# alphacep/vosk-tts

Measured on AMD Instinct MI355X. Metric: audio_samples_per_sec, higher is better.
Workload: dtype f32

## Files before the change

### vosk_tts_amd/csrc/conv_mfma.hip.h

```cpp
#pragma once
#include <type_traits>
#include <hip/hip_runtime.h>
#include <stdint.h>

typedef float f32x16 __attribute__((ext_vector_type(16)));
typedef float f32x4 __attribute__((ext_vector_type(4)));

#define CONV_CI_T 16
#define CONV_MAX_HALO 64
#define CONV_MAX_GROUPS 3

enum ConvEpilogue {
  EPI_STORE = 0,
  EPI_GATE = 1,
  EPI_RESSKIP = 2,
  EPI_COUPLE = 3,
};

struct ConvGroup {
  const float* x;
  const float* x2;
  const float* x3;
  const float* w;
  const float* w16;
  const void* wb;
  const float* bias;
  float* y;
  float* y2;
  const float* res;
  int K;
  int dil;
  int pad_l;
  int n_sg;
};

struct ConvParams {
  ConvGroup g[CONV_MAX_GROUPS];
  int n_groups;
  int B;
  int Cin;
  int x_ch_off;
  int x_ch_sign;
  long long x_bstride;
  int Tin;
  int Tin_stride;
  int M;
  int Cout;
  int Tout;
  int Tout_stride;
  long long y_bstride;
  float in_slope;
  float in_scale;
  int x_split;
  int in_mask;
  int reflect;
  const int* len;
  int relu;
  const float* scale_b;
  int scale_b_stride;
  int scale_b_off;
  int out_mask;
  const float* bias_b;
  int bias_b_stride;
  int bias_b_off;
  int ups_u;
  int ups_cout;
  int ups_shift[8];
  float* io;
  const float* u;
  float* skip;
  int H;
  int first;
  int last;
  int ntiles_m, ntiles_n;
  int xcd_mode;
  const float* dds_y2; const float* dds_g2; const float* dds_b2;
  const float* dds_sw; const float* dds_sb; const float* dds_g1; const float* dds_b1;
  float* dds_xout;
  int dds_dil;
  const float* dds_z; const float* dds_pw; const float* dds_pb;
  long long dds_z_bstride;
  const float* ln_g; const float* ln_b; const float* ln_base; const float* ln_vec;
  int ln_vec_stride, ln_vec_off;
  float* ln_out;
  const float* ln_stat_in; float* ln_stat_out; int ln_nmb;
  int row_len;
  long long* dbg;
  const int* rag;
  int rag_in_mul, rag_in_add, rag_out_mul, rag_out_add;
  int rag_tab_add;
  int rag_out_cap_add;
  int skip_len;
  const int* tile_start;
};

__device__ __forceinline__ int conv_rag_limit(int rl, int rcap, int mul, int add, int cap_add = 0) {
  const int v = rl * mul + add, c = rcap * mul + cap_add;
  return v < c ? v : c;
}

template <int BYTES>
__device__ __forceinline__ void kernarg_warm() {
  static_assert(BYTES <= 1024, "extend kernarg_warm");
  constexpr int LAST = (BYTES - 1) / 64 * 64;
#define KW_OFF(i) ((i) * 64 < LAST ? (i) * 64 : LAST)
  const unsigned long long kp = (unsigned long long)__builtin_amdgcn_kernarg_segment_ptr();
  int d;
  asm volatile(
      "s_load_dword %0, %1, %2\n s_load_dword %0, %1, %3\n s_load_dword %0, %1, %4\n s_load_dword %0, %1, %5\n"
      "s_load_dword %0, %1, %6\n s_load_dword %0, %1, %7\n s_load_dword %0, %1, %8\n s_load_dword %0, %1, %9\n"
      "s_load_dword %0, %1, %10\n s_load_dword %0, %1, %11\n s_load_dword %0, %1, %12\n s_load_dword %0, %1, %13\n"
      "s_load_dword %0, %1, %14\n s_load_dword %0, %1, %15\n s_load_dword %0, %1, %16\n s_load_dword %0, %1, %17\n"
      "s_waitcnt lgkmcnt(0)"
      : "=&s"(d)
      : "s"(kp), "n"(KW_OFF(0)), "n"(KW_OFF(1)), "n"(KW_OFF(2)), "n"(KW_OFF(3)), "n"(KW_OFF(4)), "n"(KW_OFF(5)), "n"(KW_OFF(6)),
        "n"(KW_OFF(7)), "n"(KW_OFF(8)), "n"(KW_OFF(9)), "n"(KW_OFF(10)), "n"(KW_OFF(11)), "n"(KW_OFF(12)), "n"(KW_OFF(13)),
        "n"(KW_OFF(14)), "n"(KW_OFF(15))
      : "memory");
#undef KW_OFF
}

__device__ __forceinline__ int conv_pair_mtiles(int ntiles_m, int L = blockIdx.x, int nblk = gridDim.x) {
  const int run = 8 * ntiles_m;
  if (ntiles_m < 2 || L >= (nblk / run) * run) return L;
  const int base = L / run * run, r = L - base, x = r & 7, w = r >> 3;
  return base + x * ntiles_m + w;
}
__device__ __forceinline__ bool conv_decode_block(const ConvParams& P, int& mt, int& grp, int& nt, int& b) {
  const int Lb = blockIdx.x;
  if (P.tile_start) {
    int id = conv_pair_mtiles(P.ntiles_m);
    mt = id % P.ntiles_m; id /= P.ntiles_m;
    const int total = P.tile_start[P.B];
    int q;
    if (P.n_groups > 1) { q = id % (P.ntiles_n * P.B); grp = id / (P.ntiles_n * P.B); }
    else { q = id; grp = 0; }
    if (q >= total) return false;
    int lo = 0, hi = P.B - 1;
    while (lo < hi) { const int mid = (lo + hi + 1) >> 1; if (P.tile_start[mid] <= q) lo = mid; else hi = mid - 1; }
    b = lo;
    nt = q - P.tile_start[b];
    return true;
  }
  if (P.xcd_mode == 11) {
    const int x = Lb & 7, w = Lb >> 3;
    const int per = P.ntiles_m * P.ntiles_n, n = (per - x + 7) >> 3;
    const int a = n < 32 ? n : 32;
    const int b7 = 32 - a < n ? 32 - a : n;
    int idx;
    if (w < a) { grp = 0; idx = w; }
    else if (w < a + b7) { grp = 1; idx = w - a; }
    else if (w < a + b7 + n) { grp = 2; idx = w - a - b7; }
    else if (w < a + 2 * n) { grp = 1; idx = w - a - n; }
    else { grp = 0; idx = w - 2 * n; }
    if (idx >= n) return false;
    const int t = idx * 8 + x;
    mt = t % P.ntiles_m; nt = t / P.ntiles_m;
    b = 0;
    return true;
  }
  int id;
  {
    const int nblk = gridDim.x, L = Lb;
    const int q = nblk >> 3, r = nblk & 7, xcd = L & 7, within = L >> 3;
    id = (xcd < r ? xcd * (q + 1) : r * (q + 1) + (xcd - r) * q) + within;
  }
  if (P.n_groups > 1) {
    id = P.B > 1 ? conv_pair_mtiles(P.ntiles_m) : Lb;
    mt = id % P.ntiles_m; id /= P.ntiles_m;
    nt = id % P.ntiles_n; id /= P.ntiles_n;
    b = id % P.B;
    grp = id / P.B;
  } else {
    mt = id % P.ntiles_m; id /= P.ntiles_m;
    nt = id % P.ntiles_n;
// ... 406 lines not shown
#pragma unroll
        for (int ni = 0; ni < NI; ++ni)
          acc[mi][ni] = __builtin_amdgcn_mfma_f32_32x32x2f32(a[cur][mi][p >> 2][p & 3], bv[p][ni], acc[mi][ni], 0, 0, 0);
    __builtin_amdgcn_sched_barrier(0);
  };
  using slot0 = std::integral_constant<int, 0>;
  using slot1 = std::integral_constant<int, 1>;

  for (int c = 0; c < nchunks; ++c) {
    CONV_DBG_DO(if (P.dbg) dbg_x = __builtin_readcyclecounter();)
    const float* lb = lds + (c & 1) * (CONV_CI_T * ROW) + h * ROW + wn * (NI * 32) + l31 + tap_base;
    tap(slot0{}, lb, 0);
    if (c + 1 < nchunks) load_chunk(c + 1);
    __builtin_amdgcn_sched_barrier(0);
    int kk = 1;
#pragma unroll 1
    for (; kk + 1 < K; kk += 2) {
      tap(slot1{}, lb, kk);
      tap(slot0{}, lb, kk + 1);
    }
    if (kk < K) {
      tap(slot1{}, lb, kk);
    } else {
#pragma unroll
      for (int mi = 0; mi < MI; ++mi) {
        a[0][mi][0] = a[1][mi][0];
        a[0][mi][1] = a[1][mi][1];
      }
    }
    CONV_DBG_DO(if (P.dbg) { const long long t_ = __builtin_readcyclecounter(); dbg_tap += t_ - dbg_x; dbg_x = t_; })
    if (c + 1 < nchunks) store_chunk((c + 1) & 1);
    __syncthreads();
    CONV_DBG_DO(if (P.dbg) dbg_sync += __builtin_readcyclecounter() - dbg_x;)
  }
  CONV_DBG_DO(if (P.dbg && blockIdx.x == 0 && lane == 0) {
    P.dbg[wave * 8 + 1] = dbg_tap;
    P.dbg[wave * 8 + 2] = dbg_sync;
    P.dbg[wave * 8 + 3] = __builtin_readcyclecounter() - dbg_t0;
  })

  const int lenb = (P.out_mask || EPI == EPI_RESSKIP || EPI == EPI_COUPLE) ? P.len[b] : 0x7fffffff;
  if (EPI == EPI_GATE) {
    const int j = (m0 >> 6) + wm;
#pragma unroll
    for (int ni = 0; ni < NI; ++ni)
#pragma unroll
      for (int e0 = 0; e0 < 16; e0 += 4) {
        float at[4], as[4];
#pragma unroll
        for (int i = 0; i < 4; ++i) { at[i] = acc[0][ni][e0 + i]; as[i] = acc[MI - 1][ni][e0 + i]; }
        conv_epilogue_gate<4>(P, G, b, j * 32 + 4 * h, e0, n0 + wn * (NI * 32) + ni * 32 + l31, at, as);
      }
    BT_BLOCK_END();
    return;
  }
  if (EPI == EPI_STORE && conv_epilogue_store_fast_ok(P, G)) {
    conv_epilogue_store_fragments<MI, NI>(P, G, b, lenb, m0 + wm * MI * 32, n0 + wn * (NI * 32), h, l31, acc);
    CONV_DBG_DO(if (P.dbg && blockIdx.x == 0 && lane == 0) P.dbg[wave * 8 + 4] = __builtin_readcyclecounter() - dbg_t0;)
    BT_BLOCK_END();
    return;
  }
#pragma unroll
  for (int mi = 0; mi < MI; ++mi) {
#pragma unroll
    for (int ni = 0; ni < NI; ++ni) {
#pragma unroll
      for (int e0 = 0; e0 < 16; e0 += 4) {
        float v[4];
#pragma unroll
        for (int i = 0; i < 4; ++i) v[i] = acc[mi][ni][e0 + i];
        conv_epilogue_frag<EPI, 4>(P, G, b, lenb, m0 + (wm * MI + mi) * 32 + 4 * h, e0, n0 + wn * (NI * 32) + ni * 32 + l31, v);
      }
    }
  }
  CONV_DBG_DO(if (P.dbg && blockIdx.x == 0 && lane == 0) P.dbg[wave * 8 + 4] = __builtin_readcyclecounter() - dbg_t0;)
  BT_BLOCK_END();
}

__device__ __forceinline__ float ks_ld(const float* base, unsigned byte_off) {
  return *reinterpret_cast<const float*>(reinterpret_cast<const char*>(base) + byte_off);
}
struct ks_true { static constexpr bool value = true; };
struct ks_false { static constexpr bool value = false; };
template <int MI, int NI, int EPI, int NIN, int NW>
__global__ void __launch_bounds__(NW * 64) conv_mfma_ks_kernel(const ConvParams P) {
  constexpr int M_T = MI * 32;
  constexpr int N_T = NI * 32;
  constexpr int NE = 16 / NW;
  extern __shared__ float lds[];
  kernarg_warm<sizeof(ConvParams)>();

  const int tid = threadIdx.x, lane = tid & 63;
  const int wave = __builtin_amdgcn_readfirstlane(tid >> 6);
  const int h = lane >> 5, l31 = lane & 31;
  CONV_DBG(0);
  int mt, grp, nt, b;
  if (!conv_decode_block(P, mt, grp, nt, b)) return;
  const ConvGroup& G = P.g[grp];

  const int n0 = nt * N_T, m0 = mt * M_T;
  const int K = G.K, dil = G.dil;
  int tap_base = 0;
  if (P.ups_u) tap_base = P.ups_shift[m0 / P.ups_cout];
  const int nchunks = P.Cin / CONV_CI_T;
  int t_lim = P.Tin;
  if (P.in_mask) { int lb = P.len[b]; t_lim = lb < t_lim ? lb : t_lim; }
  if (P.rag) {
    const int rl = P.rag[b], rc = P.rag[P.B];
    if (n0 >= conv_rag_limit(rl, rc, P.rag_out_mul, P.rag_out_add, P.rag_out_cap_add)) return;
    const int il = conv_rag_limit(rl, rc, P.rag_in_mul, P.rag_in_add);
    t_lim = il < t_lim ? il : t_lim;
  }
  if (P.skip_len && n0 >= P.len[b]) return;
  const float in_scale = P.in_scale, in_slope = P.in_slope;

  int tcol[NI];
#pragma unroll
  for (int ni = 0; ni < NI; ++ni) tcol[ni] = n0 + ni * 32 + l31 - G.pad_l + tap_base;
  const long long rs = (long long)P.x_ch_sign * P.Tin_stride;
  const long long ubase = (long long)b * P.x_bstride + (long long)P.x_ch_off * P.Tin_stride + (rs < 0 ? rs : 0);
  const unsigned hoff = (unsigned)(h ? (rs < 0 ? 0 : rs) : (rs < 0 ? -rs : 0));
  const float* xu = G.x + ubase;
  const float* xu2 = G.x2 ? G.x2 + ubase : nullptr;
  const float* xu3 = G.x3 ? G.x3 + ubase : nullptr;

  f32x16 acc[MI][NI];
#pragma unroll
  for (int mi = 0; mi < MI; ++mi)
#pragma unroll
    for (int ni = 0; ni < NI; ++ni)
#pragma unroll
      for (int e = 0; e < 16; ++e) acc[mi][ni][e] = 0.f;

  const int n_mblocks = P.M >> 5;
  const f32x4* wp[MI];
#pragma unroll
  for (int mi = 0; mi < MI; ++mi) {
    int mb = (m0 >> 5) + mi;
    if (mb >= n_mblocks) mb = 0;
    wp[mi] = reinterpret_cast<const f32x4*>(G.w) + (size_t)mb * G.n_sg * 64;
  }
  const int total_taps = nchunks * K;
  const int my_taps = wave < total_taps ? (total_taps - wave + NW - 1) / NW : 0;
  const int q_last = wave + NW * (my_taps > 0 ? my_taps - 1 : 0);
  const int c_last = q_last / K, k_last = q_last - c_last * K;

  constexpr int KS_U = NW >= 16 ? 1 : (NW == 8 ? (MI * NI > 1 ? 2 : 4) : 4);
  struct TapBuf {
    f32x4 a[KS_U][MI][2];
    float bq[KS_U][8][NI];
    unsigned ok[KS_U];
  };
  int lc = wave / K, lk = wave - (wave / K) * K;
  int lq = wave;
  const int step_c = NW / K, step_k = NW - step_c * K;
  const unsigned lane16 = (unsigned)lane * 16u;
  const float* xq2 = NIN > 2 ? xu2 : xu;
  const float* xq3 = NIN > 2 ? (xu3 ? xu3 : xu2) : xu;
  const float s3 = (NIN > 2 && xu3) ? 1.f : 0.f;
  const int split_chunk = NIN == 2 ? P.x_split / CONV_CI_T : 0x7fffffff;
  const int refl_t = P.reflect ? ((P.Tin > 1) ? 1 : 0) : -1;

  auto pipe_step = [&](auto has_cur, auto act, const TapBuf& cur, TapBuf& nxt) {
#pragma unroll
    for (int u = 0; u < KS_U; ++u) {
      const bool live = lq <= q_last;
      const int cc = live ? lc : c_last;
      const int kc = live ? lk : k_last;
      const int sg = 2 * (cc * K + kc);
      const bool second = NIN == 2 && cc >= split_chunk;
      const float* xsrc = second ? xu2 : xu;
      const long long coff = (long long)(second ? cc - split_chunk : cc) * CONV_CI_T * rs;
      unsigned lo[NI];
      unsigned okb = 0;
#pragma unroll
      for (int ni = 0; ni < NI; ++ni) {
        int t = tcol[ni] + kc * dil;
        t = (t == -1 && refl_t >= 0) ? refl_t : t;
        okb |= ((t >= 0) & (t < t_lim) & live) ? (1u << ni) : 0u;
        lo[ni] = (hoff + (unsigned)(t < 0 ? 0 : (t >= P.Tin ? P.Tin - 1 : t))) * 4u;
      }
      nxt.ok[u] = okb;
#pragma unroll
      for (int mi = 0; mi < MI; ++mi) {
        nxt.a[u][mi][0] = *reinterpret_cast<const f32x4*>(reinterpret_cast<const char*>(wp[mi] + (size_t)sg * 64) + lane16);
        nxt.a[u][mi][1] = *reinterpret_cast<const f32x4*>(reinterpret_cast<const char*>(wp[mi] + (size_t)(sg + 1) * 64) + lane16);
      }
#pragma unroll
      for (int p = 0; p < 8; ++p) {
        const long long ro = coff + 2 * p * rs;
#pragma unroll
        for (int ni = 0; ni < NI; ++ni) {
          float v = ks_ld(xsrc + ro, lo[ni]);
          if (NIN > 2) v = (v + ks_ld(xq2 + ro, lo[ni]) + s3 * ks_ld(xq3 + ro, lo[ni])) * in_scale;
          nxt.bq[u][p][ni] = v;
        }
        if (decltype(has_cur)::value) {
          bool okb_[NI];
#pragma unroll
          for (int ni = 0; ni < NI; ++ni) okb_[ni] = (cur.ok[u] >> ni) & 1u;
#pragma unroll
          for (int ni = 0; ni < NI; ++ni) {
            const float x_ = cur.bq[u][p][ni];
            const float bv = okb_[ni] ? (decltype(act)::value ? fmaxf(x_, x_ * in_slope) : x_) : 0.f;
#pragma unroll
            for (int mi = 0; mi < MI; ++mi)
              acc[mi][ni] = __builtin_amdgcn_mfma_f32_32x32x2f32(cur.a[u][mi][p >> 2][p & 3], bv, acc[mi][ni], 0, 0, 0);
          }
        }
        __builtin_amdgcn_sched_barrier(0);
      }
      lq += NW;
      lk += step_k;
      lc += step_c + (lk >= K ? 1 : 0);
      lk -= lk >= K ? K : 0;
    }
  };

  CONV_DBG(1);
  auto run_pipe = [&](auto act) {
    TapBuf t0, t1;
    pipe_step(ks_false{}, act, t1, t0);
#pragma unroll 1
    for (int tp = 0; tp < my_taps; tp += 2 * KS_U) {
      pipe_step(ks_true{}, act, t0, t1);
      if (tp + KS_U < my_taps) pipe_step(ks_true{}, act, t1, t0);
    }
  };
  if (my_taps > 0) {
    if (in_slope == 1.f) run_pipe(ks_false{});
    else run_pipe(ks_true{});
  }
  CONV_DBG(2);

  float* red = lds;
#pragma unroll
  for (int mi = 0; mi < MI; ++mi)
#pragma unroll
    for (int ni = 0; ni < NI; ++ni)
#pragma unroll
      for (int e = 0; e < 16; ++e) red[(((wave * MI + mi) * NI + ni) * 16 + e) * 64 + lane] = acc[mi][ni][e];
  __syncthreads();
  CONV_DBG(3);
  const int lenb = (P.out_mask || EPI == EPI_RESSKIP || EPI == EPI_COUPLE) ? P.len[b] : 0x7fffffff;
  float sum[MI][NI][NE];
#pragma unroll
  for (int mi = 0; mi < MI; ++mi)
#pragma unroll
    for (int ni = 0; ni < NI; ++ni)
#pragma unroll
      for (int ee = 0; ee < NE; ++ee) {
        const int e = NE * wave + ee;
        float a = 0.f;
#pragma unroll
        for (int w = 0; w < NW; ++w) a += red[(((w * MI + mi) * NI + ni) * 16 + e) * 64 + lane];
        sum[mi][ni][ee] = a;
      }
  CONV_DBG(4);
#pragma unroll
  for (int ni = 0; ni < NI; ++ni) {
    const int col = n0 + ni * 32 + l31;
    if (EPI == EPI_GATE) {
      conv_epilogue_gate<NE>(P, G, b, (m0 >> 6) * 32 + 4 * h, NE * wave, col, sum[0][ni], sum[MI - 1][ni]);
    } else {
#pragma unroll
      for (int mi = 0; mi < MI; ++mi) conv_epilogue_frag<EPI, NE>(P, G, b, lenb, m0 + mi * 32 + 4 * h, NE * wave, col, sum[mi][ni]);
    }
  }
  CONV_DBG(5);
}

template <typename F>
static void pack_conv_weights(float* dst, int Mpad, int Cin, int K, F src ) {
  const int n_sg = Cin / CONV_CI_T * 2 * K;
  for (int mb = 0; mb < Mpad / 32; ++mb)
    for (int sg = 0; sg < n_sg; ++sg)
      for (int lane = 0; lane < 64; ++lane)
        for (int s4 = 0; s4 < 4; ++s4) {
          const int S = sg * 4 + s4;
          const int chunk = S / (8 * K), within = S % (8 * K);
          const int kk = within / 8, p = within % 8;
          const int ci = chunk * CONV_CI_T + 2 * p + (lane >> 5);
          const int row = mb * 32 + (lane & 31);
          dst[(((size_t)mb * n_sg + sg) * 64 + lane) * 4 + s4] = src(row, ci, kk);
        }
}
```

### vosk_tts_amd/csrc/conv_small.hip.h

```cpp
#pragma once
#include "conv_mfma.hip.h"

#define C16_MAXU 20

template <typename F>
static void pack_conv_weights16(float* dst, int Mpad16, int Cin, int K, F src) {
  const int n_u = Cin / CONV_CI_T * K;
  for (int mb = 0; mb < Mpad16 / 16; ++mb)
    for (int u = 0; u < n_u; ++u)
      for (int lane = 0; lane < 64; ++lane)
        for (int q = 0; q < 4; ++q) {
          const int chunk = u / K, kk = u % K;
          const int ci = chunk * CONV_CI_T + 4 * q + (lane >> 4);
          const int row = mb * 16 + (lane & 15);
          dst[(((size_t)mb * n_u + u) * 64 + lane) * 4 + q] = src(row, ci, kk);
        }
}

static inline int c16_row_pitch(int row) { return row <= 16 ? 16 : (row <= 48 ? 48 : 80); }

#define DDS_MAXI 16
#define DDS_XP 36
__device__ __forceinline__ float c16_gelu(float v) { return 0.5f * v * (1.0f + erff(v * 0.70710678118654752440f)); }
template <int NG, int NC>
// ... 410 lines not shown
#pragma unroll
  for (int r = 0; r < 4; ++r) red[(wave * 4 + r) * 64 + lane] = acc0[r] + acc1[r];
  __syncthreads();
  if (EPI == EPI_GATE) {
    if (tid >= 128) return;
    const int ch = tid >> 4, col = n0 + (tid & 15);
    float at = 0.f, as = 0.f;
#pragma unroll
    for (int w = 0; w < NW; ++w) {
      at += red[(w * 4 + (ch & 3)) * 64 + (ch >> 2) * 16 + (tid & 15)];
      as += red[(w * 4 + (ch & 3)) * 64 + ((ch >> 2) + 2) * 16 + (tid & 15)];
    }
    const int c = mt * 8 + ch;
    const float tv = tanhf(at + ep0 + ep2);
    const float sv = 1.0f / (1.0f + __expf(-(as + ep1 + ep3)));
    if (col < P.Tout && c < P.H) G.y[(long long)b * P.y_bstride + (long long)c * P.Tout_stride + col] = tv * sv;
    return;
  }
  const bool want_stat = EPI == EPI_STORE && P.ln_stat_out != nullptr;
  if (tid >= 256 && !want_stat) return;
  const bool act = tid < 256;
  const int row = (tid >> 4) & 15, col = n0 + (tid & 15);
  float v = 0.f;
#pragma unroll
  for (int w = 0; w < NW; ++w) v += red[(w * 4 + (row & 3)) * 64 + (row >> 2) * 16 + (tid & 15)];
  const int r = m0 + row;
  const bool ok = act && col < P.Tout && r < P.Cout;
  if (!ok && !want_stat) return;
  if (EPI == EPI_STORE) {
    v += ep0;
    v += ep1;
    if (P.relu == 1) v = v > 0.f ? v : 0.f;
    else if (P.relu == 2) v = v / (1.0f + __expf(-v));
    else if (P.relu == 3) v = 0.5f * v * (1.0f + erff(v * 0.70710678118654752440f));
    if (P.out_mask && col >= lenb) v = 0.f;
    v *= ep2;
    v += ep3;
    const long long o = (long long)b * P.y_bstride + (long long)r * P.Tout_stride + col;
    if (ok) {
      G.y[o] = v;
      if (G.y2) G.y2[o] = v;
    }
    CONV_DBG(5);
    if (want_stat) {
      float* st = lds + NW * 4 * 64;
      const int nrow = P.Cout - m0 < 16 ? P.Cout - m0 : 16;
      float sv = ok ? v : 0.f;
      sv += __shfl_xor(sv, 16, 64);
      sv += __shfl_xor(sv, 32, 64);
      if (act && lane < 16) st[wave * 16 + lane] = sv;
      __syncthreads();
      const int c15 = tid & 15;
      const float mean = (st[c15] + st[16 + c15] + st[32 + c15] + st[48 + c15]) / (float)nrow;
      const float d = ok ? v - mean : 0.f;
      float q = d * d;
      q += __shfl_xor(q, 16, 64);
      q += __shfl_xor(q, 32, 64);
      __syncthreads();
      if (act && lane < 16) st[wave * 16 + lane] = q;
      __syncthreads();
      if (tid < 16 && col < P.Tout) {
        float* dst = P.ln_stat_out + (((long long)b * P.ln_nmb + mt) * P.Tout + col) * 2;
        dst[0] = mean;
        dst[1] = st[c15] + st[16 + c15] + st[32 + c15] + st[48 + c15];
      }
    }
  } else if (EPI == EPI_RESSKIP) {
    const bool to_skip = P.last || r >= P.H;
    const int sr = (P.last || r < P.H) ? r : r - P.H;
    const bool valid = col < lenb;
    float o = ep1 + v + ep0;
    if (to_skip) { if (P.last && !valid) o = 0.f; }
    else if (!valid) o = 0.f;
    float* dst = to_skip ? P.skip : P.io;
    dst[(long long)b * P.y_bstride + (long long)sr * P.Tout_stride + col] = o;
  } else {
    const long long bo = (long long)b * P.y_bstride + col;
    P.io[bo + (long long)(P.H + r) * P.Tout_stride] = col < lenb ? (ep1 - (v + ep0)) : 0.f;
    P.io[bo + (long long)r * P.Tout_stride] = ep2;
  }
}

#define WP_PITCH 96
typedef float f32x4u __attribute__((ext_vector_type(4), aligned(4)));
template <int V> struct wp_int { static constexpr int value = V; };
template <int NW, int KT>
__device__ __forceinline__ void conv_wp_body(const ConvParams& P, const ConvGroup& G, float* lds, int mt, int nt, int b, int wave, int lane) {
  constexpr int NE = 16 / NW;
  const int h = lane >> 5, l31 = lane & 31;
  const int n0 = nt * 32, m0 = mt * 32;
  const int K = KT ? KT : G.K, dil = G.dil;
  const int nchunks = P.Cin / CONV_CI_T;
  const int my_chunks = wave < nchunks ? (nchunks - wave + NW - 1) / NW : 0;
  const int last_c = wave + NW * (my_chunks > 0 ? my_chunks - 1 : 0);
  int mb = m0 >> 5;
  if (mb >= (P.M >> 5)) mb = 0;
  const f32x4* wp = reinterpret_cast<const f32x4*>(G.w) + (size_t)mb * G.n_sg * 64 + lane;
  f32x4 a[2][2];
  int lci = 0, lk = 0;
  auto load_a_half = [&](f32x4 (&d)[2], int half) {
    const int c = wave + NW * lci;
    const bool live = c <= last_c && my_chunks > 0;
    const size_t sg = 2 * ((size_t)(live ? c : last_c) * K + (live ? lk : K - 1));
    d[half] = wp[(sg + half) * 64];
    if (half) {
      ++lk;
      if (lk == K) { lk = 0; ++lci; }
    }
  };
  auto load_a = [&](f32x4 (&d)[2]) { load_a_half(d, 0); load_a_half(d, 1); };
  load_a(a[0]);
  load_a(a[1]);
  int bi = b;
  asm volatile("" : "+v"(bi));
  int len_raw = 0x7fffffff, rag_raw = 0x7fffffff;
  if (P.in_mask || P.out_mask || P.skip_len) len_raw = P.len[bi];
  int rag_cap = 0x7fffffff;
  if (P.rag) { rag_raw = P.rag[bi]; rag_cap = P.rag[P.B]; }

  const int row_len = 32 + (K - 1) * dil;
  const int nvec = (row_len + 3) >> 2;
  const bool two = nvec > 16;
  const int t_base = n0 - G.pad_l;
  const int r4 = lane >> 4, v16 = lane & 15;
  int tvp[2], tcp[2];
#pragma unroll
  for (int ps = 0; ps < 2; ++ps) {
    tvp[ps] = t_base + 4 * (v16 + 16 * ps);
    const int tc = tvp[ps] < 0 ? 0 : tvp[ps];
    tcp[ps] = tc > P.Tin - 4 ? P.Tin - 4 : tc;
  }
  const unsigned lrow = (unsigned)(r4 * P.Tin_stride);
  float* sl = lds + wave * (CONV_CI_T * WP_PITCH);
  float* sw = sl + r4 * WP_PITCH + 4 * v16;
  const float* xb = G.x + (long long)b * P.x_bstride;
  const float slope = P.in_slope;
  f32x4 v0[4], v1[4];
  const float* xb2 = G.x2 ? G.x2 + (long long)b * P.x_bstride : xb;
  const int split_chunk = P.x_split ? P.x_split / CONV_CI_T : 0x7fffffff;
  auto load_slab = [&](int ci) {
    const int c = wave + NW * ci;
    const float* xc = c >= split_chunk ? xb2 + (long long)(c - split_chunk) * CONV_CI_T * P.Tin_stride : xb + (long long)c * CONV_CI_T * P.Tin_stride;
#pragma unroll
    for (int j = 0; j < 4; ++j)
      v0[j] = *reinterpret_cast<const f32x4u*>(reinterpret_cast<const char*>(xc + 4 * j * P.Tin_stride) + (lrow + (unsigned)tcp[0]) * 4u);
    if (two) {
#pragma unroll
      for (int j = 0; j < 4; ++j)
        v1[j] = *reinterpret_cast<const f32x4u*>(reinterpret_cast<const char*>(xc + 4 * j * P.Tin_stride) + (lrow + (unsigned)tcp[1]) * 4u);
    }
  };
  if (my_chunks > 0) load_slab(0);
  const int ecol = n0 + l31;
  const int ecolc = ecol < P.Tout ? ecol : P.Tout - 1;
  long long eoff[NE];
  bool eok[NE];
  float ebias[NE], eres[NE];
#pragma unroll
  for (int i = 0; i < NE; ++i) {
    const int e = NE * wave + i;
    const int r = m0 + 4 * h + (e & 3) + 8 * (e >> 2);
    const int rc = r < P.Cout ? r : P.Cout - 1;
    eok[i] = ecol < P.Tout && r < P.Cout;
    eoff[i] = (long long)b * P.y_bstride + (long long)rc * P.Tout_stride + ecolc;
    const float bv = (G.bias ? G.bias : G.w)[rc];
    const float rv = (G.res ? G.res : G.y)[eoff[i]];
    ebias[i] = G.bias ? bv : 0.f;
// ... 168 lines not shown
```

### vosk_tts_amd/csrc/engine_convplan.hip.h

```cpp
#pragma once
struct ConvSelect {
  int force_tile = 0;
  int ks_waves = 0;
  int wp_mode = 0;
  int sp_mode = -1;
  int no_bf3 = 0;
  long env_ks_threshold = 512;
  int env_ks_shape = 0;
  long env_big_blocks = 512;
  int env_ks_waves = 0;
  int env_wp_mode = 0;
  int ks_force() const { return ks_waves ? ks_waves : env_ks_waves; }
  int wp() const { return wp_mode ? wp_mode : env_wp_mode; }
  int sp() const { return sp_mode >= 0 ? sp_mode : 1; }
};
static ConvSelect conv_select_env() {
  ConvSelect e;
  if (const char* v = getenv("VITS_KS_THRESHOLD")) e.env_ks_threshold = atol(v);
  if (const char* v = getenv("VITS_KS_SHAPE")) e.env_ks_shape = atoi(v);
  if (const char* v = getenv("VITS_BIG_BLOCKS")) e.env_big_blocks = atol(v);
  if (const char* v = getenv("VITS_KS_WAVES")) e.env_ks_waves = atoi(v);
  if (const char* v = getenv("VITS_CONV_WP")) e.env_wp_mode = atoi(v);
  return e;
}
static ConvSelect& conv_select() {
  static const ConvSelect env = conv_select_env();
  static thread_local ConvSelect sel = env;
  return sel;
}

enum ConvFamily { CONV_BIG, CONV_KS, CONV_C16, CONV_WP, CONV_SP, CONV_BF3 };
struct ConvPlan {
  ConvFamily family;
  int epi;
  int WM, WN, MI, NI;
  int NW;
  int NIN;
  int MAXU, PRO;
  int JT;
  int M_T, N_T;
};
static ConvPlan plan_big(int WM, int WN, int MI, int NI, int epi) { return {CONV_BIG, epi, WM, WN, MI, NI, WM * WN, 1, 0, 0, 0, WM * MI * 32, WN * NI * 32}; }
static ConvPlan plan_bf3(int MI, int epi) { return {CONV_BF3, epi, 2, 2, MI, 2, 4, 1, 0, 0, 0, 64 * MI, 128}; }
static ConvPlan plan_sp(int epi, int halo) { return {CONV_SP, epi, 2, 2, 1, 1, 4, 1, 0, 0, halo ? 2 : 1, 64, 64}; }
static ConvPlan plan_wp() { return {CONV_WP, EPI_STORE, 1, 1, 1, 1, 8, 1, 0, 0, 0, 32, 32}; }
static ConvPlan plan_c16_dds() { return {CONV_C16, EPI_STORE, 1, 1, 1, 1, 8, 1, 8, 1, 0, 16, 16}; }

static std::string conv_plan_name(const ConvPlan& p) {
  static const char* const epi[4] = {"STORE", "GATE", "RESSKIP", "COUPLE"};
  char b[64];
  switch (p.family) {
    case CONV_BIG: snprintf(b, sizeof b, "conv_mfma_kernel<%d,%d,%d,%d,%s>", p.WM, p.WN, p.MI, p.NI, epi[p.epi]); break;
    case CONV_KS: snprintf(b, sizeof b, "conv_mfma_ks_kernel<%d,%d,%s,%d,%d>", p.MI, p.NI, epi[p.epi], p.NIN, p.NW); break;
    case CONV_C16:
      if (p.PRO == 1) snprintf(b, sizeof b, "conv16_kernel<STORE,dds>");
      else if (p.PRO) snprintf(b, sizeof b, "conv16_kernel<STORE,ln,%d>", p.NW);
      else snprintf(b, sizeof b, "conv16_kernel<%s,%d>", epi[p.epi], p.NW);
      break;
    case CONV_WP: snprintf(b, sizeof b, "conv_wp_kernel<%d>", p.NW); break;
    case CONV_SP: snprintf(b, sizeof b, "conv_sp_kernel<%s>", epi[p.epi]); break;
    case CONV_BF3: snprintf(b, sizeof b, p.epi == EPI_GATE ? "conv_bf3_kernel<%d,GATE>" : "conv_bf3_kernel<%d>", p.MI); break;
  }
  return b;
}

static int ks_pick_waves(const ConvParams& P, long nblk, const ConvSelect& sel) {
  const int force = sel.ks_force();
  if (force == 4 || force == 8 || force == 16) return force;
  int taps = 0;
  for (int g = 0; g < P.n_groups; ++g) { const int t = P.Cin / CONV_CI_T * P.g[g].K; if (t > taps) taps = t; }
  if (nblk <= 1024 && taps >= 32) return 16;
  if (nblk <= 2048 && taps >= 16) return 8;
  return 4;
}
static int c16_waves(const ConvParams& P, int epi) {
  const ConvGroup& G = P.g[0];
  if (P.n_groups != 1 || !G.w16 || P.ups_u || G.x3 || (G.x2 && !P.x_split) || P.reflect || P.rag || P.Cin % CONV_CI_T) return 0;
  if (epi == EPI_GATE && (P.H % 8)) return 0;
  const int halo = (G.K - 1) * G.dil;
  if (halo > 48) return 0;
  if (P.ln_g && P.Cin > 8 * C16_LN_MAXC) return 0;
  if (P.ln_g && (halo > 16 || P.in_slope != 1.f || P.in_scale != 1.f || P.x_split || P.x_ch_sign != 1 || P.x_ch_off || epi != EPI_STORE)) return 0;
  const size_t lds = ((size_t)P.Cin * c16_row_pitch(16 + halo) + 16 * 32) * sizeof(float);
  if (lds > 150 * 1024) return 0;
  const int units = P.Cin / CONV_CI_T * G.K;
  if (units <= 4 * C16_MAXU) return 4;
  if (units <= 8 * C16_MAXU) return 8;
  return 0;
}
static constexpr long C16_COLS_DDS = 800;
static bool c16_dds_ok(const ConvParams& P, int dds_K, const ConvSelect& sel) {
  return (sel.force_tile == 0 || sel.force_tile == 3) && (long)P.B * P.Tout <= C16_COLS_DDS && P.g[0].w16 && P.g[0].K == 1 && P.Cin % 32 == 0 &&
         P.Cin <= 16 * DDS_MAXI && dds_K == 3 && P.Cin / CONV_CI_T <= 8 * 8 && P.len && (!P.dds_sw || P.dds_dil <= 9);
}
static bool conv_wp_ok(const ConvParams& P, int epi, int halo, bool small, const ConvSelect& sel) {
  const int mode = sel.wp();
  if (mode == 1 || epi != EPI_STORE) return false;
  if (P.x_ch_sign != 1 || P.x_ch_off || P.tile_start || P.ups_u || P.reflect || P.in_scale != 1.f || P.ln_g || P.dds_y2 || P.ln_stat_out) return false;
  if (P.Cin % CONV_CI_T || P.Tin < 4 || 32 + halo > WP_PITCH || P.in_slope < 0.f || P.in_slope > 1.f) return false;
  if (P.x_split && (P.n_groups != 1 || P.x_split % CONV_CI_T || !P.g[0].x2)) return false;
  for (int g = 0; g < P.n_groups; ++g)
    if (P.g[g].x3 || (P.g[g].x2 && !P.x_split)) return false;
  if (mode == 2) return true;
  return small && P.Cin >= 8 * CONV_CI_T && (long)P.B * P.Tout >= 256;
}
// ... 85 lines not shown
```

### vosk_tts_amd/csrc/engine_launch.hip.h

```cpp
#pragma once
static std::atomic<int> g_launch_log{0};
static std::mutex g_launch_log_mu;
static std::map<std::string, int> g_launch_counts;
struct ProfScope {
  vits_session* s; bool on; bool log; const char* op; std::string lk;
  ProfScope(vits_session* s_, const char* name, double flops, const char* kernel = "-")
      : s(s_), on(s_->profile), log(g_launch_log.load(std::memory_order_relaxed) != 0), op(name) {
    if (log) lk = kernel;
    if (!on) return;
    ProfRec r; r.name = name; r.kernel = kernel; r.flops = flops;
    hipEventCreate(&r.e0); hipEventCreate(&r.e1);
    hipEventRecord(r.e0, s->stream);
    s->prof.push_back(r);
  }
  void set_kernel(const char* k) { if (on) s->prof.back().kernel = k; if (log) lk = k; }
  ~ProfScope() {
    if (on) hipEventRecord(s->prof.back().e1, s->stream);
    if (log) { std::lock_guard<std::mutex> g(g_launch_log_mu); ++g_launch_counts[std::string(op) + "|" + lk]; }
  }
};


static bool big_lds_needed(std::atomic<unsigned long long>& done);
static void persist_launch(vits_session* s, vits_session::PersistProg& pp, const char* name, const float* d_noise = nullptr, float nsw = 0.f,
                           uint64_t seed = 0, const int64_t* d_ids = nullptr, const int* d_forced = nullptr, float length_scale = 1.f,
                           float noise_scale = 0.f) {
  vits_model* m = s->m;
  ProfScope ps(s, name, pp.flops, "persist_kernel");
  PCall c;
  c.ctl = s->ps_ctl; c.ids = reinterpret_cast<const long long*>(d_ids); c.noise = d_noise; c.nsw = nsw; c.seed = seed;
  c.solo = s->solo ? 1 : 0; c.dv = s->dv; c.item_seeds = s->item_seeds; c.trace = nullptr;
  c.dbg = m->ps_dbg;
  c.forced = d_forced; c.length_scale = length_scale; c.noise_scale = noise_scale; c.noise_prior = nullptr; c.noise_stride = 0;
  static const char* trace_path = getenv("VITS_PS_TRACE");
  static const char* trace_name = getenv("VITS_PS_TRACE_PROG");
  hipStreamCaptureStatus cap = hipStreamCaptureStatusNone;
  const bool want_trace = trace_path && !strcmp(name, trace_name ? trace_name : "dp.persist");
  if (want_trace) hipStreamIsCapturing(s->stream, &cap);
  const size_t trace_n = (size_t)m->n_cu * PS_MAX_STEPS * 8;
  if (want_trace && cap == hipStreamCaptureStatusNone) {
    hipMalloc((void**)&c.trace, trace_n * sizeof(long long));
    hipMemsetAsync(c.trace, 0, trace_n * sizeof(long long), s->stream);
  }
  g_ps_last_steps.store(pp.h.n_steps, std::memory_order_relaxed);
  if (pp.fused) hipLaunchKernelGGL(persist_kernel_fz, dim3(m->n_cu), dim3(PS_THREADS), 0, s->stream, pp.d, c);
  else hipLaunchKernelGGL(persist_kernel, dim3(m->n_cu), dim3(PS_THREADS), 0, s->stream, pp.d, c);
  if (c.trace) {
    std::vector<long long> h(trace_n);
    hipMemcpyAsync(h.data(), c.trace, trace_n * sizeof(long long), hipMemcpyDeviceToHost, s->stream);
    hipStreamSynchronize(s->stream);
    hipFree(c.trace);
    if (FILE* f = fopen(trace_path, "wb")) {
      const int hdr[4] = {m->n_cu, PS_MAX_STEPS, pp.h.n_steps, pp.h.T};
      fwrite(hdr, sizeof hdr, 1, f);
      for (int i = 0; i < pp.h.n_steps; ++i) fwrite(&pp.kinds[i], sizeof(int), 1, f);
      fwrite(h.data(), sizeof(long long), trace_n, f);
      fclose(f);
    }
  }
}

static const int* tile_table(vits_session* s, const int* len, int mul, int add, int cap, int tile, int has_cap = 0, int cap_add = 0) {
  auto key = std::make_tuple(len, mul, add + 100000 * cap_add, cap, tile);
  for (size_t i = 0; i < s->tile_keys.size(); ++i)
    if (s->tile_keys[i] == key) return s->tile_tabs + i * (s->B + 1);
  if (s->tile_keys.size() >= 32) return nullptr;
  int* tab = s->tile_tabs + s->tile_keys.size() * (s->B + 1);
  s->tile_keys.push_back(key);
  hipLaunchKernelGGL(ragged_tiles_kernel, dim3(1), dim3(64), 0, s->stream, len, s->B, mul, add, cap, tile, tab, has_cap, cap_add);
  return tab;
}

static void attach_tile_table(vits_session* s, ConvParams& P, int N_T) {
  P.tile_start = nullptr;
  if (!s || !s->arena || s->B == 1) return;
  if (P.rag) P.tile_start = tile_table(s, P.rag, P.rag_out_mul, P.rag_tab_add > P.rag_out_add ? P.rag_tab_add : P.rag_out_add, P.Tout, N_T, 1, P.rag_out_cap_add);
  else if (P.skip_len) P.tile_start = tile_table(s, P.len, 1, 0, P.Tout, N_T);
}

static bool big_lds_needed(std::atomic<unsigned long long>& done) {
  int dev = 0;
  hipGetDevice(&dev);
  const unsigned long long bit = 1ull << (dev & 63);
  return !(done.fetch_or(bit) & bit);
}
template <typename Kern>
static void launch_big_lds(Kern kern, std::atomic<unsigned long long>& done, dim3 grid, int threads, size_t lds, int lds_attr, hipStream_t st, const ConvParams& P) {
  if (lds > 64 * 1024 && big_lds_needed(done)) hipFuncSetAttribute((const void*)kern, hipFuncAttributeMaxDynamicSharedMemorySize, lds_attr);
  hipLaunchKernelGGL(kern, grid, dim3(threads), lds, st, P);
}

static int plan_grid(vits_session* s, ConvParams& P, const ConvPlan& pl, bool table) {
  if (table) attach_tile_table(s, P, pl.N_T);
  else P.tile_start = nullptr;
  P.ntiles_m = cdiv(P.M, pl.M_T);
  P.ntiles_n = cdiv(P.Tout, pl.N_T);
  return P.ntiles_m * P.ntiles_n * P.B * P.n_groups;
}
template <int WM, int WN, int MI, int NI, int EPI>
static void launch_cfg(vits_session* s, ConvParams& P, const ConvPlan& pl, int halo) {
  const int nblk = plan_grid(s, P, pl, true);
  P.row_len = pl.N_T + halo;
  const size_t lds = (size_t)2 * CONV_CI_T * P.row_len * sizeof(float);
  hipLaunchKernelGGL((conv_mfma_kernel<WM, WN, MI, NI, EPI>), dim3(nblk), dim3(WM * WN * 64), lds, s->stream, P);
}
template <int MI, int NI, int EPI, int NIN>
static void launch_ks(vits_session* s, ConvParams& P, const ConvPlan& pl) {
  const dim3 grid(plan_grid(s, P, pl, true));
  P.row_len = 0;
  const size_t lds = (size_t)pl.NW * MI * NI * 16 * 64 * sizeof(float);
  static std::atomic<unsigned long long> done16{0};
  if (pl.NW == 16) launch_big_lds(conv_mfma_ks_kernel<MI, NI, EPI, NIN, 16>, done16, grid, 16 * 64, lds, (int)lds, s->stream, P);
  else if (pl.NW == 8) hipLaunchKernelGGL((conv_mfma_ks_kernel<MI, NI, EPI, NIN, 8>), grid, dim3(8 * 64), lds, s->stream, P);
  else hipLaunchKernelGGL((conv_mfma_ks_kernel<MI, NI, EPI, NIN, 4>), grid, dim3(4 * 64), lds, s->stream, P);
}
template <int EPI, int PRO>
static void launch_c16(vits_session* s, ConvParams& P, const ConvPlan& pl) {
  const int nw = pl.NW;
  P.tile_start = nullptr;
  P.ntiles_m = cdiv(EPI == EPI_GATE ? 2 * P.H : P.Cout, 16);
  P.ntiles_n = cdiv(P.Tout, 16);
  P.row_len = c16_row_pitch(16 + (P.g[0].K - 1) * P.g[0].dil);
  size_t lds = ((size_t)P.Cin * P.row_len + (PRO == 2 ? (size_t)nw * 2 * 32 : 0)) * sizeof(float);
  lds = std::max(lds, ((size_t)nw * 4 * 64 + (P.ln_stat_out ? 64 : 0)) * sizeof(float));
  const dim3 grid(8 * cdiv(P.ntiles_m, 8) * P.ntiles_n * P.B);
  static std::atomic<unsigned long long> done[4];
  const bool few = pl.MAXU == 8;
  if (nw == 8 && few) launch_big_lds(conv16_kernel<EPI, 8, 8, PRO>, done[0], grid, 512, lds, 160 * 1024, s->stream, P);
  else if (nw == 8) launch_big_lds(conv16_kernel<EPI, 8, C16_MAXU, PRO>, done[1], grid, 512, lds, 160 * 1024, s->stream, P);
  else if (few) launch_big_lds(conv16_kernel<EPI, 4, 8, PRO>, done[2], grid, 256, lds, 160 * 1024, s->stream, P);
  else launch_big_lds(conv16_kernel<EPI, 4, C16_MAXU, PRO>, done[3], grid, 256, lds, 160 * 1024, s->stream, P);
}
static void launch_conv_wp(vits_session* s, ConvParams& P, const ConvPlan& pl) {
  int nblk = plan_grid(s, P, pl, false);
  const int per_xcd = cdiv(P.ntiles_m * P.ntiles_n, 8);
  if (P.B == 1 && P.n_groups == 3 && P.g[0].K >= P.g[1].K && P.g[1].K >= P.g[2].K && 3 * per_xcd <= 64 && per_xcd <= 32) {
    P.xcd_mode = 11;
    nblk = 8 * 3 * per_xcd;
  }
  const size_t lds = (size_t)pl.NW * CONV_CI_T * WP_PITCH * sizeof(float);
  hipLaunchKernelGGL(conv_wp_kernel<8>, dim3(nblk), dim3(pl.NW * 64), lds, s->stream, P);
}
template <int EPI>
static void launch_sp(vits_session* s, ConvParams& P, const ConvPlan& pl, int halo) {
  const dim3 grid(plan_grid(s, P, pl, true));
  P.row_len = 64 + halo;
  const size_t lds = (size_t)2 * 4 * P.row_len * SP_PITCH * sizeof(float);
  static std::atomic<unsigned long long> done1{0}, done2{0};
  if (pl.JT == 1) launch_big_lds(conv_sp_kernel<EPI, 1>, done1, grid, 256, lds, 160 * 1024, s->stream, P);
  else launch_big_lds(conv_sp_kernel<EPI, 2>, done2, grid, 256, lds, 160 * 1024, s->stream, P);
}
template <int MI, int EPI>
static void launch_bf3(vits_session* s, ConvParams& P, const ConvPlan& pl, int halo) {
  const dim3 grid(plan_grid(s, P, pl, true));
  P.row_len = 128 + halo;
  const size_t lds = (size_t)2 * 2 * P.row_len * (BF3_PITCH * 2);
  hipLaunchKernelGGL((conv_bf3_kernel<MI, EPI>), grid, dim3(256), lds, s->stream, P);
}

static void exec_conv(vits_session* s, ConvParams& P, const ConvPlan& pl, int halo) {
  const int E = pl.epi;
  switch (pl.family) {
    case CONV_BIG:
#define BIG(WM_, WN_, MI_, NI_, EPI_) \
  if (pl.WM == WM_ && pl.WN == WN_ && pl.MI == MI_ && pl.NI == NI_ && E == EPI_) return launch_cfg<WM_, WN_, MI_, NI_, EPI_>(s, P, pl, halo)
      BIG(2, 2, 1, 1, EPI_STORE); BIG(2, 2, 1, 2, EPI_STORE); BIG(2, 2, 2, 2, EPI_STORE); BIG(1, 4, 1, 1, EPI_STORE);
      BIG(2, 2, 2, 1, EPI_GATE); BIG(2, 1, 2, 1, EPI_GATE); BIG(2, 2, 1, 1, EPI_RESSKIP); BIG(2, 2, 1, 1, EPI_COUPLE);
#undef BIG
      break;
    case CONV_KS:
#define KS(MI_, NI_, EPI_, NIN_) if (pl.MI == MI_ && pl.NI == NI_ && E == EPI_ && pl.NIN == NIN_) return launch_ks<MI_, NI_, EPI_, NIN_>(s, P, pl)
      KS(1, 1, EPI_STORE, 1); KS(1, 1, EPI_STORE, 2); KS(1, 1, EPI_STORE, 3); KS(1, 2, EPI_STORE, 1); KS(1, 2, EPI_STORE, 3);
      KS(2, 1, EPI_GATE, 1); KS(1, 1, EPI_RESSKIP, 1); KS(1, 1, EPI_COUPLE, 1);
#undef KS
      break;
    case CONV_C16:
#define C16(EPI_, PRO_) if (E == EPI_ && pl.PRO == PRO_) return launch_c16<EPI_, PRO_>(s, P, pl)
      C16(EPI_STORE, 0); C16(EPI_STORE, 2); C16(EPI_STORE, 3); C16(EPI_GATE, 0); C16(EPI_RESSKIP, 0); C16(EPI_COUPLE, 0);
#undef C16
      break;
    case CONV_WP: return launch_conv_wp(s, P, pl);
    case CONV_SP:
      if (E == EPI_STORE) return launch_sp<EPI_STORE>(s, P, pl, halo);
      if (E == EPI_RESSKIP) return launch_sp<EPI_RESSKIP>(s, P, pl, halo);
      if (E == EPI_COUPLE) return launch_sp<EPI_COUPLE>(s, P, pl, halo);
      break;
    case CONV_BF3:
      if (E == EPI_GATE && pl.MI == 2) return launch_bf3<2, EPI_GATE>(s, P, pl, halo);
      if (E == EPI_STORE && pl.MI == 2) return launch_bf3<2, EPI_STORE>(s, P, pl, halo);
      if (E == EPI_STORE && pl.MI == 1) return launch_bf3<1, EPI_STORE>(s, P, pl, halo);
      break;
  }
// ... 172 lines not shown
```

Before: 48.38 million.

## Add LDS-staged channel-chunk path for 16-wave split-K conv kernel

Adds an alternative inner loop for the 16-wave split-K conv (MI=NI=1, store epilogue) in which each wave owns whole channel units. Each wave stages a leaky-ReLU'd input slab into its own LDS region and reads the B operand from it for every tap, replacing the per-tap global gathers. It is enabled by default through a VITS_KS_CHUNK env flag, but only for small grids (at most about 1.25 blocks per CU) and for kernels whose receptive row fits the 64-wide slab. The cost is more template instantiations, extra register pressure, and separate boundary and reflect handling that must match the original path.

```diff
diff --git a/vosk_tts_amd/csrc/conv_mfma.hip.h b/vosk_tts_amd/csrc/conv_mfma.hip.h
--- a/vosk_tts_amd/csrc/conv_mfma.hip.h
+++ b/vosk_tts_amd/csrc/conv_mfma.hip.h
@@ -5,6 +5,7 @@
 
 typedef float f32x16 __attribute__((ext_vector_type(16)));
 typedef float f32x4 __attribute__((ext_vector_type(4)));
+typedef float f32x4u __attribute__((ext_vector_type(4), aligned(4)));
 
 #define CONV_CI_T 16
 #define CONV_MAX_HALO 64
@@ -91,6 +92,7 @@
   int rag_tab_add;
   int rag_out_cap_add;
   int skip_len;
+  int ks_chunk;
   const int* tile_start;
 };
 
@@ -663,6 +665,139 @@
 }
 struct ks_true { static constexpr bool value = true; };
 struct ks_false { static constexpr bool value = false; };
+
+#define KS_SLAB_PITCH 64
+template <int NIN, int KT, int UP>
+__device__ __forceinline__ void ks_chunk_body(const ConvParams& P, const ConvGroup& G, float* lds, int b, int m0, int n0, int tap_base, int t_lim,
+                                              int wave, int lane, f32x16& acc) {
+  constexpr int NW = 16, ROWS = 2 * UP, NJ = ROWS / 4, NA = UP / 4, NV = NIN > 2 ? 3 : 1, D = KT ? KT : 2;
+  const int h = lane >> 5, l31 = lane & 31;
+  const int K = KT ? KT : G.K, dil = G.dil;
+  const int nunits = P.Cin / ROWS;
+  if (wave >= nunits) return;
+  const int my_units = (nunits - wave + NW - 1) / NW;
+  const int last_u = wave + NW * (my_units - 1);
+  int mb = m0 >> 5;
+  if (mb >= (P.M >> 5)) mb = 0;
+  const f32x4* wp = reinterpret_cast<const f32x4*>(G.w) + (size_t)mb * G.n_sg * 64 + lane;
+  auto load_a = [&](f32x4 (&d)[NA], int i, int ui, int tap) {
+    const int u0 = wave + NW * ui;
+    const int u = u0 <= last_u ? u0 : last_u;
+    const size_t sg = UP == 8 ? 2 * ((size_t)u * K + tap) + i : 2 * ((size_t)(u >> 1) * K + tap) + (u & 1);
+    d[i] = wp[sg * 64];
+  };
+
+  const int row_len = 32 + (K - 1) * dil;
+  const int nvec = (row_len + 3) >> 2;
+  const int t_base = n0 - G.pad_l + tap_base;
+  const int r4 = lane >> 4, v16 = lane & 15;
+  const int tv = t_base + 4 * v16;
+  const int tc0 = tv < 0 ? 0 : tv;
+  const int tc = tc0 > P.Tin - 4 ? P.Tin - 4 : tc0;
+  const long long rs = (long long)P.x_ch_sign * P.Tin_stride;
+  const long long ars = rs < 0 ? -rs : rs;
+  const unsigned loff = ((unsigned)((rs < 0 ? 3 - r4 : r4) * ars) + (unsigned)tc) * 4u;
+  const long long ubase = (long long)b * P.x_bstride + (long long)P.x_ch_off * P.Tin_stride + (rs < 0 ? 3 * rs : 0);
+  const float* xu = G.x + ubase;
+  const float* xu2 = G.x2 ? G.x2 + ubase : xu;
+  const float* xu3 = G.x3 ? G.x3 + ubase : xu2;
+  const float s3 = (NIN > 2 && G.x3) ? 1.f : 0.f;
+  const int split_unit = NIN == 2 ? P.x_split / ROWS : 0x7fffffff;
+  const float in_scale = P.in_scale, slope = P.in_slope;
+  const int refl_t = P.reflect ? ((P.Tin > 1) ? 1 : 0) : -1;
+  float* sl = lds + wave * (16 * KS_SLAB_PITCH);
+  float* sw = sl + r4 * KS_SLAB_PITCH + 4 * v16;
+  f32x4 v[NV][NJ];
+  auto load_slab = [&](int ui) {
+    const int u = wave + NW * ui;
+    const bool second = NIN == 2 && u >= split_unit;
+    const long long co = (long long)(second ? u - split_unit : u) * ROWS * rs;
+    const float* src[3] = {(second ? xu2 : xu) + co, xu2 + co, xu3 + co};
+#pragma unroll
+    for (int n = 0; n < NV; ++n)
+#pragma unroll
+      for (int j = 0; j < NJ; ++j) v[n][j] = *reinterpret_cast<const f32x4u*>(reinterpret_cast<const char*>(src[n] + 4 * j * rs) + loff);
+  };
+  load_slab(0);
+  __builtin_amdgcn_sched_barrier(0);
+  f32x4 a[D][NA];
+#pragma unroll
+  for (int t = 0; t < D; ++t)
+#pragma unroll
+    for (int i = 0; i < NA; ++i) load_a(a[t], i, 0, t < K ? t : K - 1);
+  const bool interior = t_base >= 0 && t_base + 4 * nvec <= t_lim;
+  auto stage = [&]() {
+    if (v16 >= nvec) return;
+#pragma unroll
+    for (int j = 0; j < NJ; ++j) {
+      f32x4 x = v[0][j], o;
+      if (NIN > 2) x = (x + v[1][j] + s3 * v[2][j]) * in_scale;
+      if (interior) {
+#pragma unroll
+        for (int q = 0; q < 4; ++q) o[q] = fmaxf(x[q], x[q] * slope);
+      } else {
+#pragma unroll
+        for (int q = 0; q < 4; ++q) {
+          const int t = tv + q, te = (t == -1 && refl_t >= 0) ? refl_t : t, idx = te - tc;
+          const float e = idx <= 0 ? x[0] : (idx == 1 ? x[1] : (idx == 2 ? x[2] : x[3]));
+          o[q] = (te >= 0 && te < t_lim) ? fmaxf(e, e * slope) : 0.f;
+        }
+      }
+      *reinterpret_cast<f32x4*>(sw + 4 * j * KS_SLAB_PITCH) = o;
+    }
+  };
+  const float* bl = sl + h * KS_SLAB_PITCH + l31;
+  auto read_b = [&](float (&d)[UP], int tap) {
+#pragma unroll
+    for (int p = 0; p < UP; ++p) d[p] = bl[2 * p * KS_SLAB_PITCH + tap * dil];
+  };
+  auto mfma4 = [&](const f32x4& w, const float (&d)[UP], int p0) {
+#pragma unroll
+    for (int p = 0; p < 4; ++p) acc = __builtin_amdgcn_mfma_f32_32x32x2f32(w[p], d[p0 + p], acc, 0, 0, 0);
+  };
+#pragma unroll 1
+  for (int ui = 0; ui < my_units; ++ui) {
+    stage();
+    if (ui == 0) CONV_DBG(6);
+    if (ui + 1 < my_units) load_slab(ui + 1);
+    float bb[2][UP];
+    read_b(bb[0], 0);
+    if (KT) {
+#pragma unroll
+      for (int tap = 0; tap < (KT ? KT : 1); ++tap) {
+        if (tap + 1 < KT) read_b(bb[(tap + 1) & 1], tap + 1);
+        __builtin_amdgcn_sched_barrier(0);
+#pragma unroll
+        for (int i = 0; i < NA; ++i) {
+          mfma4(a[tap][i], bb[tap & 1], 4 * i);
+          load_a(a[tap], i, ui + 1, tap);
+        }
+        __builtin_amdgcn_sched_barrier(0);
+      }
+    } else {
+#pragma unroll 1
+      for (int tap = 0; tap < K; tap += 2) {
+        read_b(bb[1], tap + 1 < K ? tap + 1 : tap);
+#pragma unroll
+        for (int i = 0; i < NA; ++i) mfma4(a[0][i], bb[0], 4 * i);
+#pragma unroll
+        for (int i = 0; i < NA; ++i) load_a(a[0], i, tap + 2 < K ? ui : ui + 1, tap + 2 < K ? tap + 2 : tap + 2 - K);
+        if (tap + 1 < K) {
+          read_b(bb[0], tap + 2 < K ? tap + 2 : tap + 1);
+#pragma unroll
+          for (int i = 0; i < NA; ++i) mfma4(a[1][i], bb[1], 4 * i);
+#pragma unroll
+          for (int i = 0; i < NA; ++i) load_a(a[1], i, tap + 3 < K ? ui : ui + 1, tap + 3 < K ? tap + 3 : tap + 3 - K);
+        }
+      }
+      if (K & 1) {
+#pragma unroll
+        for (int i = 0; i < NA; ++i) { const f32x4 t = a[0][i]; a[0][i] = a[1][i]; a[1][i] = t; }
+      }
+    }
+  }
+}
+
 template <int MI, int NI, int EPI, int NIN, int NW>
 __global__ void __launch_bounds__(NW * 64) conv_mfma_ks_kernel(const ConvParams P) {
   constexpr int M_T = MI * 32;
@@ -713,6 +848,30 @@
 #pragma unroll
       for (int e = 0; e < 16; ++e) acc[mi][ni][e] = 0.f;
 
+  bool chunked = false;
+  if constexpr (NW == 16 && MI == 1 && NI == 1 && EPI == EPI_STORE) {
+    if (P.ks_chunk) {
+      chunked = true;
+      f32x16 part;
+#pragma unroll
+      for (int e = 0; e < 16; ++e) part[e] = 0.f;
+      bool whole = false;
+      if constexpr (NIN < 3) whole = nchunks >= NW;
+      if (whole) {
+        if constexpr (NIN < 3) {
+          if (K == 4) ks_chunk_body<NIN, 4, 8>(P, G, lds, b, m0, n0, tap_base, t_lim, wave, lane, part);
+          else if (K == 7) ks_chunk_body<NIN, 7, 8>(P, G, lds, b, m0, n0, tap_base, t_lim, wave, lane, part);
+          else ks_chunk_body<NIN, 0, 8>(P, G, lds, b, m0, n0, tap_base, t_lim, wave, lane, part);
+        }
+      } else {
+        if (K == 4) ks_chunk_body<NIN, 4, 4>(P, G, lds, b, m0, n0, tap_base, t_lim, wave, lane, part);
+        else if (K == 7) ks_chunk_body<NIN, 7, 4>(P, G, lds, b, m0, n0, tap_base, t_lim, wave, lane, part);
+        else ks_chunk_body<NIN, 0, 4>(P, G, lds, b, m0, n0, tap_base, t_lim, wave, lane, part);
+      }
+#pragma unroll
+      for (int e = 0; e < 16; ++e) lds[(wave * 16 + e) * 64 + lane] = part[e];
+    }
+  }
   const int n_mblocks = P.M >> 5;
   const f32x4* wp[MI];
 #pragma unroll
@@ -808,19 +967,21 @@
       if (tp + KS_U < my_taps) pipe_step(ks_true{}, act, t1, t0);
     }
   };
-  if (my_taps > 0) {
+  if (!chunked && my_taps > 0) {
     if (in_slope == 1.f) run_pipe(ks_false{});
     else run_pipe(ks_true{});
   }
   CONV_DBG(2);
 
   float* red = lds;
-#pragma unroll
-  for (int mi = 0; mi < MI; ++mi)
-#pragma unroll
-    for (int ni = 0; ni < NI; ++ni)
-#pragma unroll
-      for (int e = 0; e < 16; ++e) red[(((wave * MI + mi) * NI + ni) * 16 + e) * 64 + lane] = acc[mi][ni][e];
+  if (!chunked) {
+#pragma unroll
+    for (int mi = 0; mi < MI; ++mi)
+#pragma unroll
+      for (int ni = 0; ni < NI; ++ni)
+#pragma unroll
+        for (int e = 0; e < 16; ++e) red[(((wave * MI + mi) * NI + ni) * 16 + e) * 64 + lane] = acc[mi][ni][e];
+  }
   __syncthreads();
   CONV_DBG(3);
   const int lenb = (P.out_mask || EPI == EPI_RESSKIP || EPI == EPI_COUPLE) ? P.len[b] : 0x7fffffff;
diff --git a/vosk_tts_amd/csrc/conv_small.hip.h b/vosk_tts_amd/csrc/conv_small.hip.h
--- a/vosk_tts_amd/csrc/conv_small.hip.h
+++ b/vosk_tts_amd/csrc/conv_small.hip.h
@@ -516,7 +516,6 @@
 }
 
 #define WP_PITCH 96
-typedef float f32x4u __attribute__((ext_vector_type(4), aligned(4)));
 template <int V> struct wp_int { static constexpr int value = V; };
 template <int NW, int KT>
 __device__ __forceinline__ void conv_wp_body(const ConvParams& P, const ConvGroup& G, float* lds, int mt, int nt, int b, int wave, int lane) {
diff --git a/vosk_tts_amd/csrc/engine_convplan.hip.h b/vosk_tts_amd/csrc/engine_convplan.hip.h
--- a/vosk_tts_amd/csrc/engine_convplan.hip.h
+++ b/vosk_tts_amd/csrc/engine_convplan.hip.h
@@ -10,6 +10,7 @@
   long env_big_blocks = 512;
   int env_ks_waves = 0;
   int env_wp_mode = 0;
+  int env_ks_chunk = 1;
   int ks_force() const { return ks_waves ? ks_waves : env_ks_waves; }
   int wp() const { return wp_mode ? wp_mode : env_wp_mode; }
   int sp() const { return sp_mode >= 0 ? sp_mode : 1; }
@@ -21,6 +22,7 @@
   if (const char* v = getenv("VITS_BIG_BLOCKS")) e.env_big_blocks = atol(v);
   if (const char* v = getenv("VITS_KS_WAVES")) e.env_ks_waves = atoi(v);
   if (const char* v = getenv("VITS_CONV_WP")) e.env_wp_mode = atoi(v);
+  if (const char* v = getenv("VITS_KS_CHUNK")) e.env_ks_chunk = atoi(v);
   return e;
 }
 static ConvSelect& conv_select() {
diff --git a/vosk_tts_amd/csrc/engine_launch.hip.h b/vosk_tts_amd/csrc/engine_launch.hip.h
--- a/vosk_tts_amd/csrc/engine_launch.hip.h
+++ b/vosk_tts_amd/csrc/engine_launch.hip.h
@@ -104,10 +104,18 @@
   const size_t lds = (size_t)2 * CONV_CI_T * P.row_len * sizeof(float);
   hipLaunchKernelGGL((conv_mfma_kernel<WM, WN, MI, NI, EPI>), dim3(nblk), dim3(WM * WN * 64), lds, s->stream, P);
 }
+static bool ks_chunk_takes(const vits_session* s, const ConvParams& P, const ConvPlan& pl, long nblk) {
+  const ConvGroup& G = P.g[0];
+  if (!conv_select().env_ks_chunk || pl.NW != 16 || pl.MI != 1 || pl.NI != 1 || pl.epi != EPI_STORE || P.n_groups != 1) return false;
+  if (G.K < 4 || G.dil < 1 || 32 + (G.K - 1) * G.dil > KS_SLAB_PITCH || P.Tin < 4) return false;
+  const long cus = s->m->n_cu > 0 ? s->m->n_cu : 256;
+  return 4 * nblk <= 5 * cus;
+}
 template <int MI, int NI, int EPI, int NIN>
 static void launch_ks(vits_session* s, ConvParams& P, const ConvPlan& pl) {
   const dim3 grid(plan_grid(s, P, pl, true));
   P.row_len = 0;
+  P.ks_chunk = ks_chunk_takes(s, P, pl, (long)grid.x) ? 1 : 0;
   const size_t lds = (size_t)pl.NW * MI * NI * 16 * 64 * sizeof(float);
   static std::atomic<unsigned long long> done16{0};
   if (pl.NW == 16) launch_big_lds(conv_mfma_ks_kernel<MI, NI, EPI, NIN, 16>, done16, grid, 16 * 64, lds, (int)lds, s->stream, P);
```

New measurement: 48.89 million (median of 6 runs). 1.01x the previous value.
